# PrimeIntellect-ai/protocol

Measured on AMD Instinct MI355X. Metric: task x worker pair-evals/sec (full-swarm match), higher is better.
Workload: dtype u64

## Files before the change

protocol_amd/csrc/pm_device.h:

```cpp
#ifndef PM_DEVICE_H
#define PM_DEVICE_H

#include <hip/hip_runtime.h>
#include <stdint.h>

#include "pm_engine.h"

namespace pm {

static constexpr double PM_RAD = 3.14159265358979323846 / 180.0;
static constexpr uint64_t PM_KEY_NOLOC = 0x7FEFFFFFFFFFFFFFull;
static constexpr double PM_A_MAX_SAFE = 1.0 - 1.0 / 1048576.0;
static constexpr double PM_A_CHORD_MIN = 1.3e-6;
static constexpr uint32_t PM_CARVE_SLOTS = 8192;
static constexpr uint32_t PM_CARVE_PART = 64;
static constexpr uint32_t PM_CARVE_SEL_CAP = 256;
static constexpr uint32_t PM_CARVE_SLOT_BITS = 13;
static constexpr uint32_t PM_CARVE_BIG_SLOTS = 262144;
static constexpr uint32_t PM_CARVE_SLOT_BITS_BIG = 18;
static constexpr uint32_t PM_CARVE_SLOT_BITS_MEM = 21;
static constexpr double PM_TIE_BAND = 1.0 / 68719476736.0;
static constexpr double PM_TIE_BAND_BIG = 1.0 / 2147483648.0;
static constexpr double PM_TIE_BAND_MEM = 1.0 / 268435456.0;
static constexpr uint32_t PM_PROP_ROW = 96;
// ... 35 lines not shown
       SC_FINISH = 50,
       SC_FINISH_TICKET = 52,
       SC_TRACE = 51,
       SC_BATCHES = 54
};
static constexpr uint32_t PM_STREAM_TRACE_CAP = 1u << 17;
enum { SROW_NONE = 0, SROW_BITMAP = 1, SROW_WALK = 2, SROW_SWEEP = 3 };

struct CompatArgs {
  uint32_t W, n_cfgs, model_words;
  const uint32_t *flags, *gpu_count, *gpu_mem, *gpu_cls, *cpu_cores, *ram, *storage;
  const pm_config_row* cfgs;
  const pm_gpu_alt_row* alts;
  const uint32_t* model_bits;
  uint64_t* compat;
};

enum : uint32_t {
  REP_WHY = 0,
  REP_IDLE = PM_WHY_N,
  REP_GROUPS,
  REP_MEMBERS,
  REP_NO_TASK,
  REP_TASKS,
  REP_STRIDE = 16
};

struct ReportArgs {
  CompatArgs c;
  const int32_t* group_of;
// ... 196 lines not shown
  uint32_t stage_cap_g, stage_cap_m;
  uint32_t *stage_cfg, *stage_n, *stage_off, *stage_mem;
  unsigned long long* g_id_out;
  uint32_t* g_task_out;
  CarveStatus* h_status;
  unsigned long long* stream_trace;
  uint32_t n_avail, start_ci;
  uint32_t avail_cfg[PM_MAX_CONFIGS];
  uint32_t min_size[PM_MAX_CONFIGS];
  uint32_t max_size[PM_MAX_CONFIGS];
  uint32_t *g_cfg, *g_n, *g_off, *members;
  uint32_t cap_groups, cap_members;
  CarveStatus* status;
};

void launch_compat(const CompatArgs& a, hipStream_t s);
void launch_explain(const CompatArgs& p, const uint32_t* rows, uint32_t n, uint32_t stride, uint32_t* why_out, hipStream_t s);
void launch_config_report(const ReportArgs& a, uint32_t max_blocks, hipStream_t s);
void launch_task_report(const ReportArgs& a, uint32_t max_blocks, hipStream_t s);
void launch_group_spread(const SpreadArgs& a, hipStream_t s);
void launch_config_spread(const pm_group_spread_row* rows, const uint32_t* row_cfg, uint32_t n_rows, uint32_t n_cfgs,
                          SpreadCfgAcc* out, uint32_t max_blocks, hipStream_t s);
void launch_nearest(const NearArgs& a, hipStream_t s);
void launch_geo(const double* lat, const double* lon, double* coslat, double* ux, double* uy, double* uz, uint32_t W,
                hipStream_t s);
void launch_triad(const double* b, const double* c, double* a, size_t n, hipStream_t s);
#ifdef PM_ROW_BENCH
hipError_t launch_row_bench(const CarveArgs* d_args, uint32_t seed, uint32_t ci, uint32_t reps, uint32_t mode, unsigned long long* d_out, hipStream_t s);
#endif
void launch_row_network_test(const uint64_t* keys, const uint32_t* sites, uint32_t n_waves, uint32_t n_per_wave, uint32_t slot_bits,
                             uint64_t ulps, uint32_t upto, uint64_t* rows_out, uint32_t* mismatches, hipStream_t s);
// ... 1 lines not shown
void launch_distance_key_test(const double* in, const double* geo, uint32_t n, uint32_t mode, double* out, hipStream_t s);
void launch_update_rows(const RowUpdateArgs& a, hipStream_t s);
void launch_worker_selector(const int32_t* group_of, const uint32_t* g_cfg, uint32_t R, const uint32_t* rows,
                            uint64_t* sel, hipStream_t s);
void launch_eligible_selector(const uint32_t* wflags, const int32_t* group_of, const uint64_t* compat,
                              uint64_t enabled, uint32_t W, const uint8_t* shard, uint32_t my_rank, uint64_t* sel,
                              hipStream_t s);
void launch_chooser_rank(const int32_t* group_of, const uint64_t* g_id, const uint32_t* count, uint32_t R,
                         const uint32_t* rows, uint64_t seed, uint32_t* rank, hipStream_t s);
void launch_table_scatter(const pm_assignment* x, const uint32_t* xrow, uint32_t W, pm_assignment* table,
                          uint32_t* task_col, uint32_t* g_task_next, const uint64_t* t_live, const uint32_t* t_prefix,
                          hipStream_t s);
void launch_group_rank(const int32_t* group_of, const uint32_t* g_n, const uint32_t* g_off, const uint32_t* members,
                       const uint32_t* addr_rank, uint32_t W, uint32_t* rank_in_group, uint32_t* by_rank,
                       hipStream_t s);
void launch_claim_publish(const ClaimArgs& a, hipStream_t s);
void launch_match_prep(const MatchPrepArgs& a, hipStream_t s);
void launch_build_planes(const uint64_t* col_mask, uint32_t n_cols, uint32_t c_begin, uint32_t c_end, uint32_t stride,
                         uint32_t n_planes, uint64_t* planes, hipStream_t s);
void launch_pair_sweep(int variant, const uint64_t* row_sel, uint32_t R, const uint64_t* col_mask,
                       const uint64_t* planes, uint32_t c_begin, uint32_t c_end, uint32_t stride, uint32_t n_planes,
                       uint32_t* first, uint32_t* count, hipStream_t s, bool inited = false);
void launch_pair_select(int variant, const uint64_t* row_sel, uint32_t R, const uint64_t* col_mask,
                        const uint64_t* planes, uint32_t c_begin, uint32_t c_end, uint32_t stride, uint32_t n_planes,
                        const uint32_t* rank, uint32_t* out, hipStream_t s);
void launch_task_prefix(const uint64_t* live, uint32_t w_begin, uint32_t w_end, uint32_t* prefix, hipStream_t s);
void launch_task_delete(const uint32_t* slots, uint32_t n, uint64_t* tmask, uint64_t* live, uint64_t* planes,
                        uint32_t stride, uint32_t n_planes, hipStream_t s);
void launch_task_intern(const uint64_t* tmask, const uint64_t* live, uint32_t u_begin, uint32_t u_end, uint64_t valid,
                        uint64_t* keys, uint32_t n_slots, uint32_t* vals, uint32_t* counter_and_overflow, uint64_t* umask,
                        uint32_t cap_u, hipStream_t s);
// ... 3 lines not shown
                               uint32_t* count_out, hipStream_t s);
void launch_task_compact(const uint32_t* first_u, const uint32_t* count_u, uint32_t u_begin, uint32_t u_end,
                         const uint64_t* live, const uint32_t* prefix, uint32_t* first_out, uint32_t* count_out,
                         hipStream_t s);
void launch_newest(const int64_t* created_at, const uint64_t* live, uint32_t t_begin, uint32_t t_end,
                   uint32_t* idx_by_block, long long* val_by_block, uint32_t n_blocks, hipStream_t s);
void launch_group_ids(uint64_t* g_id, uint32_t* g_task, uint32_t n, uint64_t rng_state, hipStream_t s);
hipError_t carve_kernels_init();
hipError_t launch_carve(const CarveArgs* d_args, uint32_t flags, uint32_t start_ci, size_t lds_bytes, hipStream_t s);
uint32_t launch_carve_prep(const CarveArgs* d_args, uint32_t W, hipStream_t s);
hipError_t launch_carve_args_put(const CarveArgs& a, CarveArgs* d_args, hipStream_t s);
uint32_t launch_carve_elig(CarveArgs* d_args, const CarveArgs* put, uint32_t W, uint32_t n_bound, uint32_t index_min, uint32_t start_ci,
                           bool fresh, uint32_t n_groups0, uint32_t n_members0, hipStream_t s);
void launch_carve_apply(const CarveArgs* d_args, uint32_t W, hipStream_t s);
void launch_carve_propose(const CarveArgs* d_args, uint32_t W, hipStream_t s);
hipError_t launch_carve_stream(const CarveArgs* d_args, uint32_t start_ci, uint32_t n_prop_wgs, hipStream_t s);
void launch_scatter_const(uint32_t* dst, const uint32_t* idx, uint32_t n, uint32_t v, hipStream_t s);
void launch_scatter_pairs(uint32_t* dst, const uint32_t* pairs, uint32_t n, hipStream_t s);
void launch_merge_place(const CarveArgs* d_args, uint32_t n_order, uint32_t n_groups0, uint32_t n_members0, uint32_t steps0,
                        hipStream_t s);

}
#endif
```

protocol_amd/csrc/pm_engine_carve.inc:

```
static int32_t ensure_compat(pm_engine* e, hipEvent_t end_ev = nullptr) {
  if (!e->have_cfgs || !e->have_workers) return set_error(PM_ESTATE, "configs and workers must be uploaded first");
  {
    int32_t rcf = sync_flags(e);
    if (rcf) return rcf;
  }
  if (!e->compat_dirty) return PM_OK;
  for (const pm_gpu_alt_row& a : e->alts)
    if ((a.flags & PM_G_MODEL) && a.model_row >= e->model_rows)
      return set_error(PM_ESTATE, "a GPU alternative names a model row but pm_set_model_table was not called");
  if (e->model_rows && e->cls_check_dirty)
    for (uint32_t w = 0; w < e->W; ++w)
      if ((e->h_flags[w] & PM_W_GPU_MODEL) && e->h_gpu_cls[w] >= e->model_classes)
        return set_error(PM_ERANGE, "worker gpu_model_class outside the model table");
  e->cls_check_dirty = false;
  HIPCHK(e->d_compat.ensure(std::max<size_t>(e->W, 1)));
  CompatArgs a{};
  a.W = e->W;
  a.n_cfgs = uint32_t(e->cfgs.size());
  a.model_words = (e->model_classes + 31u) / 32u;
  a.flags = e->d_flags.p;
  a.gpu_count = e->d_gpu_count.p;
  a.gpu_mem = e->d_gpu_mem.p;
  a.gpu_cls = e->d_gpu_cls.p;
  a.cpu_cores = e->d_cpu_cores.p;
  a.ram = e->d_ram.p;
  a.storage = e->d_storage.p;
  a.cfgs = e->d_cfgs.p;
  a.alts = e->d_alts.p;
  a.model_bits = e->d_model_bits.p;
  a.compat = e->d_compat.p;
  HIPCHK(hipEventRecord(e->kev[0], e->stream));
  launch_compat(a, e->stream);
  HIPCHK(hipEventRecord(end_ev ? end_ev : e->kev[1], e->stream));
  HIPCHK(hipGetLastError());
  e->k_compat_recorded = true;
  e->k_compat_end = end_ev ? end_ev : e->kev[1];
  e->compat_dirty = false;
  e->h_compat_valid = false;
  return PM_OK;
}

static int32_t pull_compat(pm_engine* e) {
  if (e->h_compat_valid) return PM_OK;
  e->h_compat.resize(e->W);
  if (e->W) {
    HIPCHK(hipMemcpyAsync(e->h_compat.data(), e->d_compat.p, size_t(e->W) * 8, hipMemcpyDeviceToHost, e->stream));
    HIPCHK(hipStreamSynchronize(e->stream));
  }
  e->h_compat_valid = true;
  return PM_OK;
}
// ... 275 lines not shown
struct FormRun {
  CarveArgs a;
  CarveStatus st;
  std::vector<uint32_t> avail;
  uint32_t g0 = 0, m0 = 0, start_ci = 0;
  size_t lds = 0;
  bool use_props = false;
  bool nothing = false;
  uint32_t n_bound = 0;
  uint32_t n_elig_hint = 0;
  bool stream = false;
  uint32_t stream_wgs = 0;
  bool rearmed = false;
  uint32_t stage_cap = 0;
  bool args_pending = false;
};

static int32_t launch_propose_timed(pm_engine* e, const CarveArgs* d_args, uint32_t n_bound, hipStream_t s);

static int32_t form_setup_args(pm_engine* e, FormRun* r);

static int32_t form_queue_init(pm_engine* e, FormRun* r, bool fresh = false) {
  fresh = fresh && r->use_props;
  if (!fresh) HIPCHK(hipMemcpyAsync(e->d_status.p, &r->st, sizeof(r->st), hipMemcpyHostToDevice, e->stream));
  if (r->use_props) {
    if (!r->stream) HIPCHK(hipMemsetAsync(e->d_desc.p, 0, sizeof(BatchDesc), e->stream));
    const uint32_t index_min = !r->a.prune_mode ? 0u : r->a.prune_mode >= 2u ? 1u : PM_CELL_AUTO_N;
    if (r->stream) {
      if (e->stream_seq == 0 || e->stream_seq >= 127) {
        HIPCHK(hipMemsetAsync(e->d_stream_sq.p, 0, size_t(PM_STREAM_SQ) * 8, e->stream));
// ... 3 lines not shown
      }
      e->stream_seq += 1;
      const uint32_t tag0 = e->stream_seq << 25;
      if (r->a.stream_tag0 != tag0) {
        r->a.stream_tag0 = tag0;
        if (!r->args_pending)
          HIPCHK(hipMemcpyAsync(&e->d_carve_args.p->stream_tag0, &r->a.stream_tag0, sizeof(uint32_t), hipMemcpyHostToDevice, e->stream));
      }
    }
    e->tick_carve_launches += launch_carve_elig(e->d_carve_args.p, r->args_pending ? &r->a : nullptr, e->W, r->n_bound,
                                                r->n_elig_hint >= index_min ? index_min : 0u, r->start_ci, fresh, r->st.n_groups,
                                                r->st.n_members, e->stream);
    r->args_pending = false;
    host_mark("form: eligible list queued");
    if (r->stream) {
      HIPCHK(launch_carve_stream(e->d_carve_args.p, r->start_ci, r->stream_wgs, e->stream));
      e->tick_carve_launches += 2;
      return PM_OK;
    }
    e->tick_carve_launches += launch_carve_prep(e->d_carve_args.p, r->n_bound, e->stream);
    HIPCHK(hipGetLastError());
  } else
    HIPCHK(launch_carve(e->d_carve_args.p, CARVE_F_INIT | CARVE_F_RUN | CARVE_F_ALL, r->start_ci, r->lds, e->stream));
  e->tick_carve_launches++;
  return PM_OK;
}

static int32_t form_begin(pm_engine* e, FormRun* r, hipEvent_t begin_ev = nullptr) {
  int32_t rc = absorb_groups(e);
  if (rc) return rc;
  rc = ensure_compat(e);
// ... 292 lines not shown
```

protocol_amd/csrc/pm_engine_groups.inc:

```

template <typename T>
static int32_t upload(DevBuf<T>& d, const T* src, size_t n, hipStream_t s) {
  HIPCHK(d.ensure(n ? n : 1));
  if (n) HIPCHK(hipMemcpyAsync(d.p, src, n * sizeof(T), hipMemcpyHostToDevice, s));
  return PM_OK;
}

static void pub_clear(pm_engine* e) {
  const int cur = e->pub_cur.load(std::memory_order_relaxed);
  if (cur < 0) return;
  PubTable& t = e->pub[cur];
  const uint64_t s0 = t.seq.load(std::memory_order_relaxed);
  t.seq.store(s0 + 1, std::memory_order_relaxed);
  std::atomic_thread_fence(std::memory_order_release);
  t.cleared.store(1u, std::memory_order_relaxed);
  t.seq.store(s0 + 2, std::memory_order_release);
}

static void reset_groups_locked(pm_engine* e) {
  e->groups.clear();
  e->n_dead_groups = 0;
  e->absorb_pending = false;
  e->h_group_of.assign(e->W, -1);
  e->id_rng = e->cfg.group_id_seed;
// ... 40 lines not shown

static int32_t delta_stage(pm_engine* e, int which, size_t n) {
  HIPCHK(hipStreamSynchronize(e->stream));
  if (e->h_delta_cap[which] < n) {
    if (e->h_delta_pin[which]) (void)hipHostFree(e->h_delta_pin[which]);
    e->h_delta_pin[which] = nullptr;
    e->h_delta_cap[which] = 0;
    const size_t cap = n + n / 2 + 4096;
    HIPCHK(hipHostMalloc((void**)&e->h_delta_pin[which], cap * sizeof(uint32_t)));
    e->h_delta_cap[which] = cap;
  }
  HIPCHK(e->d_delta[which].ensure(n));
  return PM_OK;
}

static int32_t push_groups(pm_engine* e) {
  if (!e->groups_dirty) return PM_OK;
  const size_t room_g = std::min(e->d_g_cfg.cap, std::min(e->d_g_task.cap, std::min(e->d_g_task_next.cap, e->d_g_id.cap)));
  const size_t room_m = std::min(e->d_members.cap, std::min(e->d_by_rank.cap, e->d_rank_in_group.cap));
  if (e->groups_delta_ok && e->n_dead_groups * 4 <= e->groups.size() + 256 && size_t(e->d_n_groups) + e->W <= room_g &&
      size_t(e->d_n_members) + e->W <= room_m && e->d_n_groups == e->groups.size()) {
    HIPCHK(e->d_group_of.grow_keep(std::max<size_t>(e->W, 1), e->delta_tail_from == PM_NONE ? e->W : e->delta_tail_from, e->stream));
    if (e->delta_tail_from != PM_NONE && e->delta_tail_from < e->W)
      HIPCHK(hipMemsetAsync(e->d_group_of.p + e->delta_tail_from, 0xFF, size_t(e->W - e->delta_tail_from) * 4, e->stream));
    if (!e->delta_free.empty()) {
      const size_t n = e->delta_free.size();
      int32_t rc = delta_stage(e, 0, n);
      if (rc) return rc;
      std::memcpy(e->h_delta_pin[0], e->delta_free.data(), n * 4);
      HIPCHK(hipMemcpyAsync(e->d_delta[0].p, e->h_delta_pin[0], n * 4, hipMemcpyHostToDevice, e->stream));
      launch_scatter_const(reinterpret_cast<uint32_t*>(e->d_group_of.p), e->d_delta[0].p, uint32_t(n), 0xFFFFFFFFu, e->stream);
// ... 29 lines not shown
  HIPCHK(e->d_g_id.ensure(capG));
  HIPCHK(e->d_members.ensure(capM));
  HIPCHK(e->d_by_rank.ensure(capM));
  HIPCHK(e->d_rank_in_group.ensure(capM));
  HIPCHK(e->d_group_of.ensure(capM));
  if (G) {
    HIPCHK(hipMemcpyAsync(e->d_g_cfg.p, g_cfg.data(), G * 4, hipMemcpyHostToDevice, e->stream));
    HIPCHK(hipMemcpyAsync(e->d_g_n.p, g_n.data(), G * 4, hipMemcpyHostToDevice, e->stream));
    HIPCHK(hipMemcpyAsync(e->d_g_off.p, g_off.data(), G * 4, hipMemcpyHostToDevice, e->stream));
    HIPCHK(hipMemcpyAsync(e->d_g_task.p, g_task.data(), G * 4, hipMemcpyHostToDevice, e->stream));
    HIPCHK(hipMemcpyAsync(e->d_g_id.p, g_id.data(), G * 8, hipMemcpyHostToDevice, e->stream));
  }
  if (!members.empty())
    HIPCHK(hipMemcpyAsync(e->d_members.p, members.data(), members.size() * 4, hipMemcpyHostToDevice, e->stream));
  if (e->W) {
    if (G == 0)
      HIPCHK(hipMemsetAsync(e->d_group_of.p, 0xFF, size_t(e->W) * 4, e->stream));
    else
      HIPCHK(hipMemcpyAsync(e->d_group_of.p, e->h_group_of.data(), size_t(e->W) * 4, hipMemcpyHostToDevice, e->stream));
  }
  if (G) HIPCHK(hipStreamSynchronize(e->stream));
  e->d_n_groups = uint32_t(G);
  e->d_n_members = uint32_t(members.size());
  e->groups_dirty = false;
  e->groups_delta_ok = true;
  e->delta_free.clear();
  e->delta_tail_from = PM_NONE;
  return PM_OK;
}

static int32_t sync_flags(pm_engine* e) {
// ... 25 lines not shown
```

protocol_amd/csrc/pm_engine_match.inc:

```

static int32_t ensure_task_planes(pm_engine* e) {
  if (!e->have_tasks) return set_error(PM_ESTATE, "tasks must be uploaded first");
  const uint32_t n_planes = uint32_t(e->cfgs.size());
  const uint32_t stride = e->t_cap / 64u;
  if (e->tplanes_dirty) {
    HIPCHK(e->d_tplanes.ensure(std::max<size_t>(size_t(stride) * (n_planes + 1), 1)));
    launch_build_planes(e->d_tmask.p, e->t_cap, e->t_lo, e->t_cap, stride, n_planes, e->d_tplanes.p, e->stream);
    HIPCHK(hipGetLastError());
    e->tplanes_dirty = false;
  }
  if (e->tprefix_dirty) {
    launch_task_prefix(e->d_tlive.p, e->t_lo / 64u, stride, e->d_tprefix.p, e->stream);
    HIPCHK(hipGetLastError());
    e->tprefix_dirty = false;
  }
  return PM_OK;
}

static uint32_t task_position(pm_engine* e, uint32_t u) {
  if (u == PM_NONE || u < e->t_lo || u >= e->t_cap) return PM_NONE;
  if (!e->h_tprefix_valid) {
    const uint32_t stride = e->t_cap / 64u;
    e->h_tprefix.assign(stride, 0);
    uint32_t acc = 0;
// ... 34 lines not shown
  if (!n_app) return PM_OK;
  const uint64_t bit = 1ull << cfg;
  uint32_t r = 0;
  if (e->cfg.chooser == PM_CHOOSE_SEEDED) r = uint32_t(splitmix64_mix(e->cfg.chooser_seed ^ group_id) % n_app);
  for (uint32_t u = e->t_lo; u < e->t_cap; ++u)
    if (e->h_tmask[u] & bit) {
      if (r == 0) {
        *task_out = u;
        return PM_OK;
      }
      --r;
    }
  return PM_OK;
}

static int32_t run_match(pm_engine* e, bool want_count, std::vector<uint32_t>* count_out, bool dist = false, size_t G_ub = 0) {
  pm_assignment* const claim_h_table = dist ? nullptr : e->claim_h_table;
  uint32_t* const claim_h_gtask = dist ? nullptr : e->claim_h_gtask;
  e->claim_h_table = nullptr;
  e->claim_h_gtask = nullptr;
  if (!e->have_cfgs || !e->have_workers || !e->have_tasks)
    return set_error(PM_ESTATE, "configs, workers and tasks must be uploaded first");
  int32_t rc = push_groups(e);
  if (rc) return rc;
  const int variant = int(e->cfg.sweep_variant);
  host_mark("match: groups pushed");
  rc = ensure_task_planes(e);
  if (rc) return rc;
  host_mark("match: task planes");
  const uint32_t R = dist ? uint32_t(e->h_own_rows.size()) : e->W;
  const uint32_t* rows = dist ? e->d_own_rows.p : nullptr;
  rc = ensure_sweep_outputs(e, R);
  if (rc) return rc;
  HIPCHK(e->d_sel.ensure(std::max<uint32_t>(e->W, 1)));
  HIPCHK(e->d_table.ensure(std::max<uint32_t>(e->W, 1)));
  HIPCHK(e->d_task_col.ensure(std::max<uint32_t>(e->W, 1)));
  if (e->W == 0) return PM_OK;
  const uint32_t n_planes = uint32_t(e->cfgs.size());

  host_mark("match: selector launch");
  const size_t G = G_ub ? G_ub : e->d_n_groups;
  if (!dist) {
    MatchPrepArgs m{};
    m.W = e->W;
    m.G = uint32_t(G);
    m.group_of = e->d_group_of.p;
    m.g_cfg = e->d_g_cfg.p;
    m.g_n = e->d_g_n.p;
    m.g_off = e->d_g_off.p;
    m.members = e->d_members.p;
    m.addr_rank = e->d_addr_rank.p;
    m.g_task = e->d_g_task.p;
// ... 33 lines not shown
  c.group_of = e->d_group_of.p;
  c.g_n = e->d_g_n.p;
  c.g_off = e->d_g_off.p;
  c.g_task = e->d_g_task.p;
  c.g_id = e->d_g_id.p;
  c.g_task_next = e->d_g_task_next.p;
  c.chosen = chosen;
  c.rank_in_group = e->d_rank_in_group.p;
  c.by_rank = e->d_by_rank.p;
  c.t_live = e->d_tlive.p;
  c.t_prefix = e->d_tprefix.p;
  c.table = dist ? e->d_table_x.p + size_t(e->dist_rank) * e->dist_cap_t : e->d_table.p;
  c.task_col = e->d_task_col.p;
  c.h_table = claim_h_table;
  c.h_gtask = claim_h_gtask;
  launch_claim_publish(c, e->stream);
  HIPCHK(hipGetLastError());
  if (want_count && count_out) {
    count_out->resize(R);
    HIPCHK(hipMemcpyAsync(count_out->data(), e->d_count.p, size_t(R) * 4, hipMemcpyDeviceToHost, e->stream));
  }
  return PM_OK;
}

static int32_t pub_buffer(pm_engine* e, PubTable& t, uint32_t rows, uint64_t** out) {
  uint64_t* words = t.words.load(std::memory_order_relaxed);
  if (t.cap_rows < rows || !words) {
    const size_t cap = std::max<size_t>(size_t(rows) + rows / 8 + 64, 64);
    uint64_t* nw = nullptr;
    if (hipHostMalloc((void**)&nw, cap * 32) != hipSuccess || !nw)
      return set_error(PM_ENOMEM, "out of pinned host memory for the published table");
// ... 206 lines not shown
```

protocol_amd/csrc/pm_engine_state.inc:

```
struct pm_engine {
  pm_engine_config cfg{};
  hipStream_t stream = nullptr;
  hipStream_t stream_owned = nullptr;
  bool own_stream = true;
  hipEvent_t ev[6]{};
  hipEvent_t kev[6]{};
  hipEvent_t k_carve_begin = nullptr;
  hipEvent_t k_compat_end = nullptr;
  bool one_event_behind_carve = false;
  float k_ms_compat = 0, k_ms_carve = 0, k_ms_sweep = 0;
  bool k_sweep_recorded = false, k_compat_recorded = false;
  std::chrono::steady_clock::time_point tick_t0{};
  bool end_event_queued = false;
  uint64_t tick_cand_sum = 0;
  unsigned long long carve_prof[64]{};
  unsigned long long carve_why[25]{};
  uint32_t debug_mem_above = 0;
  uint32_t debug_abort_after = 0;
  uint32_t delta_pushes = 0;
  uint32_t merge_streamed = 0;
  uint32_t merge_stream_min = 512;
  uint32_t prune_mode = 1;
  uint32_t prune_factor = 512;
  uint32_t walk_cap_div = 0;
// ... 162 lines not shown
```

protocol_amd/csrc/pm_engine_tick.inc:

```
static void tick_reset(pm_engine* e) {
  e->tick_host_resolved = e->tick_carve_launches = e->tick_carve_steps = 0;
  e->tick_fast_steps = 0;
  e->tick_cand_sum = 0;
  e->tick_props = 0;
  e->tick_prop_keys = 0;
  e->tick_stream_timeouts = e->tick_stream_tickets = e->tick_stream_aborts = 0;
  e->k_ms_propose = 0;
  e->prop_ev_used = 0;
  e->k_ms_compat = e->k_ms_carve = e->k_ms_sweep = 0;
  e->k_sweep_recorded = e->k_compat_recorded = false;
  e->one_event_behind_carve = false;
  e->end_event_queued = false;
  e->tick_t0 = std::chrono::steady_clock::now();
}

static int32_t tick_stats(pm_engine* e, pm_stats* stats, uint32_t n_formed, uint32_t n_merged) {
  if (!e->end_event_queued) HIPCHK(hipEventRecord(e->ev[5], e->stream));
  HIPCHK(hipEventSynchronize(e->ev[5]));
  hipEvent_t const sweep_end = e->end_event_queued ? e->ev[5] : e->ev[4];
  pm_stats s{};
  HIPCHK(hipEventElapsedTime(&s.ms_compat, e->ev[0], e->ev[1]));
  HIPCHK(hipEventElapsedTime(&s.ms_carve, e->ev[1], e->ev[2]));
  if (e->one_event_behind_carve) {
    s.ms_merge = 0.0f;
    HIPCHK(hipEventElapsedTime(&s.ms_sweep, e->ev[2], sweep_end));
  } else {
    HIPCHK(hipEventElapsedTime(&s.ms_merge, e->ev[2], e->ev[3]));
    HIPCHK(hipEventElapsedTime(&s.ms_sweep, e->ev[3], sweep_end));
  }
  if (!e->end_event_queued) HIPCHK(hipEventElapsedTime(&s.ms_publish, e->ev[4], e->ev[5]));
  if (e->end_event_queued)
    s.ms_total = std::chrono::duration<float, std::milli>(std::chrono::steady_clock::now() - e->tick_t0).count();
  else
    HIPCHK(hipEventElapsedTime(&s.ms_total, e->ev[0], e->ev[5]));
  if (e->k_compat_recorded) HIPCHK(hipEventElapsedTime(&s.ms_compat_kernel, e->kev[0], e->k_compat_end ? e->k_compat_end : e->kev[1]));
  if (e->k_sweep_recorded) HIPCHK(hipEventElapsedTime(&s.ms_sweep_kernel, e->kev[4], e->kev[5]));
  s.ms_carve_kernel = e->k_ms_carve;
  s.carve_cand_sum = e->tick_cand_sum;
  s.ms_propose_kernel = e->k_ms_propose;
  s.proposals = e->tick_props;
  s.propose_keys = e->tick_prop_keys;
  s.n_groups = uint32_t(e->groups.size() - e->n_dead_groups);
  s.n_formed = n_formed;
  s.n_merged = n_merged;
  s.carve_steps = e->tick_carve_steps;
  s.carve_fast_steps = e->tick_fast_steps;
  s.host_resolved_steps = e->tick_host_resolved;
  s.carve_launches = e->tick_carve_launches;
  s.pair_evals = uint64_t(e->T) * uint64_t(e->W);
  e->last_stats = s;
// ... 1 lines not shown
  return PM_OK;
}

int32_t pm_tick(pm_engine* e, pm_stats* stats) {
  if (!e) return set_error(PM_EINVAL, "null argument");
  std::lock_guard<std::mutex> lk(e->mu);
  if (e->dist_phase != 0) return set_error(PM_ESTATE, "a stepwise tick is in progress");
  HIPCHK(hipSetDevice(e->cfg.device));
  if (!e->have_cfgs || !e->have_workers || !e->have_tasks)
    return set_error(PM_ESTATE, "configs, workers and tasks must be uploaded first");
  if (e->dist_world > 1) return set_error(PM_ESTATE, "multi-GPU engine: use the stepwise tick (pm_dist_tick_begin ...)");
  if (e->dist_phase != 0) return set_error(PM_ESTATE, "a stepwise tick is in progress");
  tick_reset(e);
  host_mark("tick: begin");
  uint32_t n_formed = 0, n_merged = 0;
  HIPCHK(hipEventRecord(e->ev[0], e->stream));
  e->compat_dirty = true;
  int32_t rc = absorb_groups(e);
  if (rc) return rc;
  rc = push_groups(e);
  if (rc) return rc;
  rc = ensure_task_planes(e);
  if (rc) return rc;
  rc = ensure_compat(e, e->ev[1]);
  if (rc) return rc;
  if (!e->k_compat_recorded) HIPCHK(hipEventRecord(e->ev[1], e->stream));
  host_mark("tick: compat queued");
  FormRun r;
  rc = form_begin(e, &r, e->ev[1]);
  if (rc) return rc;
  bool done = false;
  if (r.stream && !r.nothing && !e->tick_needs_merge) {
    PubRun pr;
    HIPCHK(hipEventRecord(e->ev[2], e->stream));
    const size_t G_ub = std::min<size_t>(size_t(r.g0) + r.stage_cap, std::min(e->d_g_task.cap, e->d_g_task_next.cap));
    host_mark("tick: carve queued");
    rc = publish_open(e, &pr, G_ub);
    if (rc) return rc;
    host_mark("tick: snapshot buffer open");
    rc = run_match(e, false, nullptr, false, G_ub);
    if (rc) {
      publish_abandon(e, pr);
      return rc;
    }
    HIPCHK(hipEventRecord(e->ev[5], e->stream));
    e->end_event_queued = true;
    host_mark("tick: everything queued");
    if (hipEventSynchronize(e->ev[2]) != hipSuccess) {
      publish_abandon(e, pr);
      return set_error(PM_ENODEV, "tick: the stream failed");
    }
    host_mark("tick: carve through");
    const CarveStatus& hs = *e->h_status;
    size_t solo = hs.n_solo;
    for (const Group& g : e->groups) solo += g.members.size() == 1 && !g.dead;
    const bool fits = hs.n_groups >= r.g0 && hs.n_groups - r.g0 <= r.stage_cap && hs.n_members >= r.m0 &&
                      hs.n_members - r.m0 <= r.stage_cap && hs.n_groups <= G_ub;
    if (hs.state == CARVE_STATE_DONE && fits && solo < 2) {
      r.st = hs;
      rc = form_finish(e, &r, &n_formed, false, true);
// ... 170 lines not shown
```

protocol_amd/csrc/pm_kernels.hip:

```cpp
#include <hip/hip_runtime.h>
#include <stdint.h>

#include "pm_device.h"

#if defined(__HIP_DEVICE_COMPILE__) && !defined(__gfx950__)
#error "pm_kernels.hip is written for gfx950 (MI355X): see the note on the placement kernels' fences above"
#endif

namespace pm {


template <int CTRL, int ROW_MASK>
__device__ __forceinline__ uint32_t dpp_add_step(uint32_t v) {
  return v + (uint32_t)__builtin_amdgcn_update_dpp(0, (int)v, CTRL, ROW_MASK, 0xF, false);
}
__device__ __forceinline__ uint32_t wave_incl_scan_u32(uint32_t v) {
  v = dpp_add_step<0x111, 0xF>(v);
  v = dpp_add_step<0x112, 0xF>(v);
  v = dpp_add_step<0x114, 0xF>(v);
  v = dpp_add_step<0x118, 0xF>(v);
  v = dpp_add_step<0x142, 0xA>(v);
  v = dpp_add_step<0x143, 0xC>(v);
  return v;
}
// ... 91 lines not shown
      }
      if ((cfg.flags & PM_R_RAM) && (!(wf & PM_W_RAM) || wram < cfg.ram_mb)) ok = false;
      if ((cfg.flags & PM_R_STORAGE) && (!(wf & PM_W_STORAGE) || wsto < cfg.storage_gb)) ok = false;
      if (cfg.alt_count) {
        bool any = false;
        if (wf & PM_W_HAS_GPU)
          for (uint32_t k = 0; k < cfg.alt_count; ++k)
            any |= gpu_alt_meets(wf, wcount, wmem, wcls, p.alts[cfg.alt_begin + k], p.model_bits, p.model_words);
        ok = ok && any;
      }
    }
    mask |= (uint64_t)ok << c;
  }
  if (!SLICED) {
    p.compat[w] = mask;
    return;
  }
  s_part[threadIdx.x] = mask;
  __syncthreads();
  if (slice == 0u && in) p.compat[w] = s_part[lane] | s_part[64u + lane] | s_part[128u + lane] | s_part[192u + lane];
}
__global__ __launch_bounds__(256) void compat_kernel(CompatArgs p) { compat_body<false>(p); }
__global__ __launch_bounds__(256) void compat_sliced_kernel(CompatArgs p) { compat_body<true>(p); }

__global__ __launch_bounds__(256) void triad_kernel(const double* __restrict__ b, const double* __restrict__ c,
                                                    double* __restrict__ a, size_t n) {
  for (size_t i = (size_t)blockIdx.x * 256u + threadIdx.x; i < n; i += (size_t)gridDim.x * 256u) a[i] = b[i] + 3.0 * c[i];
}

__device__ __forceinline__ void geo_of(double la, double lo, double* coslat, double* ux, double* uy, double* uz) {
  const double phi = la * PM_RAD, lam = lo * PM_RAD;
  const double c = cos(phi);
  *coslat = c;
  *ux = c * cos(lam);
  *uy = c * sin(lam);
// ... 530 lines not shown
```

protocol_amd/csrc/pm_launch.inc:

```

void launch_compat(const CompatArgs& a, hipStream_t s) {
  if (a.W == 0) return;
  if (a.W < 65536u)
    hipLaunchKernelGGL(compat_sliced_kernel, dim3((a.W + 63u) / 64u), dim3(256), 0, s, a);
  else
    hipLaunchKernelGGL(compat_kernel, dim3((a.W + 255u) / 256u), dim3(256), 0, s, a);
}
void launch_triad(const double* b, const double* c, double* a, size_t n, hipStream_t s) {
  hipLaunchKernelGGL(triad_kernel, dim3(256 * 32), dim3(256), 0, s, b, c, a, n);
}
void launch_row_network_test(const uint64_t* keys, const uint32_t* sites, uint32_t n_waves, uint32_t n_per_wave, uint32_t slot_bits,
                             uint64_t ulps, uint32_t upto, uint64_t* rows_out, uint32_t* mismatches, hipStream_t s) {
  hipLaunchKernelGGL(row_network_test_kernel, dim3(n_waves / 4u), dim3(256), 0, s, keys, sites, n_per_wave, slot_bits, ulps, upto, rows_out,
                     mismatches);
}
void launch_distance_key_test(const double* in, const double* geo, uint32_t n, uint32_t mode, double* out, hipStream_t s) {
  if (n == 0) return;
  hipLaunchKernelGGL(distance_key_test_kernel, dim3((n + 255u) / 256u), dim3(256), 0, s, in, geo, n, mode, out);
}
void launch_geo(const double* lat, const double* lon, double* coslat, double* ux, double* uy, double* uz, uint32_t W,
                hipStream_t s) {
  if (W == 0) return;
  hipLaunchKernelGGL(geo_kernel, dim3((W + 255u) / 256u), dim3(256), 0, s, lat, lon, coslat, ux, uy, uz, W);
}
// ... 26 lines not shown
  hipLaunchKernelGGL(table_scatter_kernel, dim3((W + 255u) / 256u), dim3(256), 0, s, x, xrow, W, table, task_col,
                     g_task_next, t_live, t_prefix);
}
void launch_group_rank(const int32_t* group_of, const uint32_t* g_n, const uint32_t* g_off, const uint32_t* members,
                       const uint32_t* addr_rank, uint32_t W, uint32_t* rank_in_group, uint32_t* by_rank,
                       hipStream_t s) {
  if (W == 0) return;
  hipLaunchKernelGGL(group_rank_kernel, dim3((W + 255u) / 256u), dim3(256), 0, s, group_of, g_n, g_off, members,
                     addr_rank, W, rank_in_group, by_rank);
}
void launch_match_prep(const MatchPrepArgs& a, hipStream_t s) {
  const uint32_t n = a.W > a.G ? a.W : a.G;
  if (n == 0) return;
  hipLaunchKernelGGL(match_prep_kernel, dim3((n + 255u) / 256u), dim3(256), 0, s, a);
}
void launch_claim_publish(const ClaimArgs& a, hipStream_t s) {
  if (a.R == 0) return;
  hipLaunchKernelGGL(claim_publish_kernel, dim3((a.R + 255u) / 256u), dim3(256), 0, s, a);
}

void launch_build_planes(const uint64_t* col_mask, uint32_t n_cols, uint32_t c_begin, uint32_t c_end, uint32_t stride,
                         uint32_t n_planes, uint64_t* planes, hipStream_t s) {
  const uint32_t w0 = c_begin / 64u, w1 = (c_end + 63u) / 64u;
  if (w1 <= w0) return;
  hipLaunchKernelGGL(build_planes_kernel, dim3(((w1 - w0) * 64u + 255u) / 256u), dim3(256), 0, s, col_mask, n_cols, w0,
                     w1, stride, n_planes, planes);
}

void launch_pair_sweep(int variant, const uint64_t* row_sel, uint32_t R, const uint64_t* col_mask,
                       const uint64_t* planes, uint32_t c_begin, uint32_t c_end, uint32_t stride, uint32_t n_planes,
                       uint32_t* first, uint32_t* count, hipStream_t s, bool inited) {
  if (R == 0) return;
  const uint32_t rb = (R + 255u) / 256u;
// ... 209 lines not shown
```

protocol_amd/csrc/pm_stream.inc:

```

enum { SLW_TREQ = PM_STREAM_TP,
       SLW_PAY,
       SLW_TISSUED,
       SLW_SCANW, SLW_SCANLO, SLW_SCANHI,
       SLW_TIMEOUTS,
       SLW_LA,
       SLW_TEND,
       SLW_ACKT, SLW_ACKP0, SLW_ACKP1, SLW_ACKP2, SLW_ACKP3, SLW_ACKP4,
       SLW_NCAND,
       SLW_P_CI, SLW_P_CI1, SLW_P_PAY, SLW_P_PAY1, SLW_P_MAX, SLW_P_MAX1, SLW_P_T0, SLW_P_T01, SLW_P_CNT, SLW_P_CNT1,
       SLW_P_SCANW, SLW_P_SCANW1, SLW_P_SCANLO, SLW_P_SCANLO1, SLW_P_SCANHI, SLW_P_SCANHI1,
       SLW_WORDS };
static_assert(SLW_TREQ == PM_STREAM_SLW_TREQ && SLW_PAY == PM_STREAM_SLW_PAY, "the words carve_fast_steps reads");
static_assert(SLW_WORDS <= PM_STREAM_TP + 32u, "ticket state fits its LDS region");
#ifndef STREAM_NPARK
#define STREAM_NPARK 5u
#endif
#ifndef STREAM_PARK_NB
#define STREAM_PARK_NB 16u
#endif
#ifndef STREAM_NAP_TICKETER
#define STREAM_NAP_TICKETER 4
#endif
#ifndef STREAM_NAP_PARK
// ... 2106 lines not shown
    st->fast_steps += c.fast_steps;
    st->slow_steps += c.steps - c.fast_steps;
    st->n_batches += 1u;
    if (n > 0u && n <= PM_CARVE_BIG_SLOTS) {
      st->stream_timeouts += sl_words[SLW_TIMEOUTS];
      st->stream_tickets += sl_words[SLW_TISSUED];
    }
  }
}

__global__ __launch_bounds__(256) void carve_finish_kernel(const CarveArgs* __restrict__ pa) {
  const CarveArgs& p = *pa;
  const auto st = G(p.status);
  const auto ctl = G(p.stream_ctl);
  __shared__ uint32_t s_last;
  if (ctl[SC_FINISH]) {
    const uint32_t g_lo = st->g_lo, g_hi = st->g_hi;
    const uint32_t total = gridDim.x * 256u;
    const uint32_t id_g0 = p.id_g0, m0 = p.stage_m0, cap_g = p.stage_cap_g, cap_m = p.stage_cap_m;
    const bool stage = p.stage_cfg != nullptr;
    uint32_t solo = 0;
    for (uint32_t g = g_lo + blockIdx.x * 256u + threadIdx.x; g < g_hi; g += total) {
      const uint32_t off = G(p.g_off)[g], gn = G(p.g_n)[g];
      const uint32_t k = g - id_g0;
      for (uint32_t j = 0; j < gn; ++j) {
        const uint32_t w = G(p.order)[G(p.members)[off + j]];
        G(p.members)[off + j] = w;
        if (p.mode == CARVE_MODE_FORM) G(p.group_of)[w] = (int32_t)g;
        if (stage && off + j - m0 < cap_m) p.stage_mem[off + j - m0] = w;
      }
      if (p.g_id_out) {
        unsigned long long z = p.id_state + (unsigned long long)(k + 1u) * 0x9E3779B97F4A7C15ull;
        z = (z ^ (z >> 30)) * 0xBF58476D1CE4E5B9ull;
        z = (z ^ (z >> 27)) * 0x94D049BB133111EBull;
        p.g_id_out[g] = z ^ (z >> 31);
        p.g_task_out[g] = PM_NONE;
      }
      if (stage && k < cap_g) {
        p.stage_cfg[k] = G(p.g_cfg)[g];
        p.stage_n[k] = gn;
        p.stage_off[k] = off;
      }
      solo += gn == 1u ? 1u : 0u;
    }
    solo = wave_sum(solo);
    if ((threadIdx.x & 63u) == 0u && solo) atomicAdd(&p.status->n_solo, solo);
  }
  if (!p.h_status) return;
  __syncthreads();
  if (threadIdx.x == 0) {
    __threadfence();
    s_last = atomicAdd(&p.stream_ctl[SC_FINISH_TICKET], 1u);
  }
  __syncthreads();
  if (s_last != gridDim.x - 1u) return;
  const auto src = G((const uint32_t*)p.status);
  uint32_t* dst = (uint32_t*)p.h_status;
  for (uint32_t k = threadIdx.x; k < (uint32_t)(sizeof(CarveStatus) / 4u); k += 256u) dst[k] = ld_ag32((const stream_gu32*)(src + k));
}

hipError_t launch_carve_stream(const CarveArgs* d_args, uint32_t start_ci, uint32_t n_prop_wgs, hipStream_t s) {
  hipLaunchKernelGGL(carve_stream_kernel, dim3(1u + n_prop_wgs), dim3(CARVE_THREADS), PM_STREAM_LDS_BYTES, s, d_args, start_ci);
  hipLaunchKernelGGL(carve_finish_kernel, dim3(128), dim3(256), 0, s, d_args);
  return hipGetLastError();
}

#ifdef PM_ROW_BENCH
__global__ __launch_bounds__(CARVE_THREADS) void carve_row_bench_kernel(const CarveArgs* __restrict__ pa, uint32_t s, uint32_t ci, uint32_t reps,
                                                                        unsigned long long* __restrict__ out) {
  const CarveArgs& p = *pa;
  extern __shared__ __attribute__((aligned(16))) unsigned char s_raw[];
  const uint32_t lane = threadIdx.x & 63u, wave = threadIdx.x >> 6;
  if (wave != 0u) return;
  const auto st = G((const CarveStatus*)p.status);
  const uint32_t n = st->n_eligible;
  if (n == 0u || n > PM_CARVE_BIG_SLOTS || s >= n) return;
  const uint32_t SB = n > PM_CARVE_SLOTS ? PM_CARVE_SLOT_BITS_BIG : PM_CARVE_SLOT_BITS;
  const double TIE_BAND = n > PM_CARVE_SLOTS ? PM_TIE_BAND_BIG : PM_TIE_BAND;
// ... 42 lines not shown
```

Measured before the change: 1130 billion.

## Fold group_of reset into compat kernel, attach events to launches, parallelize member finish

The separate memset that resets group_of to -1 is folded into the compat kernel, and standalone hipEventRecord calls are replaced by events attached to hipExtLaunchKernelGGL launches, cutting commands on the stream per tick. The carve finish kernel also moves member remapping from a per-group serial loop to a per-member loop, where each block locates its group by cooperative binary search over g_off. This balances work when group sizes vary, at the cost of extra searches and block barriers. The ev[0] record now moves to the compat launch, so the total-time window measured from ev[0] shrinks.

```diff
diff --git a/protocol_amd/csrc/pm_device.h b/protocol_amd/csrc/pm_device.h
--- a/protocol_amd/csrc/pm_device.h
+++ b/protocol_amd/csrc/pm_device.h
@@ -73,6 +73,7 @@
   const pm_gpu_alt_row* alts;
   const uint32_t* model_bits;
   uint64_t* compat;
+  int32_t* group_of_fill;
 };
 
 enum : uint32_t {
@@ -299,7 +300,7 @@
   CarveStatus* status;
 };
 
-void launch_compat(const CompatArgs& a, hipStream_t s);
+bool launch_compat(const CompatArgs& a, hipStream_t s, hipEvent_t start_ev = nullptr, hipEvent_t stop_ev = nullptr);
 void launch_explain(const CompatArgs& p, const uint32_t* rows, uint32_t n, uint32_t stride, uint32_t* why_out, hipStream_t s);
 void launch_config_report(const ReportArgs& a, uint32_t max_blocks, hipStream_t s);
 void launch_task_report(const ReportArgs& a, uint32_t max_blocks, hipStream_t s);
@@ -331,7 +332,7 @@
 void launch_group_rank(const int32_t* group_of, const uint32_t* g_n, const uint32_t* g_off, const uint32_t* members,
                        const uint32_t* addr_rank, uint32_t W, uint32_t* rank_in_group, uint32_t* by_rank,
                        hipStream_t s);
-void launch_claim_publish(const ClaimArgs& a, hipStream_t s);
+bool launch_claim_publish(const ClaimArgs& a, hipStream_t s, hipEvent_t stop_ev = nullptr);
 void launch_match_prep(const MatchPrepArgs& a, hipStream_t s);
 void launch_build_planes(const uint64_t* col_mask, uint32_t n_cols, uint32_t c_begin, uint32_t c_end, uint32_t stride,
                          uint32_t n_planes, uint64_t* planes, hipStream_t s);
@@ -365,7 +366,7 @@
                            bool fresh, uint32_t n_groups0, uint32_t n_members0, hipStream_t s);
 void launch_carve_apply(const CarveArgs* d_args, uint32_t W, hipStream_t s);
 void launch_carve_propose(const CarveArgs* d_args, uint32_t W, hipStream_t s);
-hipError_t launch_carve_stream(const CarveArgs* d_args, uint32_t start_ci, uint32_t n_prop_wgs, hipStream_t s);
+hipError_t launch_carve_stream(const CarveArgs* d_args, uint32_t start_ci, uint32_t n_prop_wgs, hipStream_t s, hipEvent_t finish_ev = nullptr);
 void launch_scatter_const(uint32_t* dst, const uint32_t* idx, uint32_t n, uint32_t v, hipStream_t s);
 void launch_scatter_pairs(uint32_t* dst, const uint32_t* pairs, uint32_t n, hipStream_t s);
 void launch_merge_place(const CarveArgs* d_args, uint32_t n_order, uint32_t n_groups0, uint32_t n_members0, uint32_t steps0,
diff --git a/protocol_amd/csrc/pm_engine_carve.inc b/protocol_amd/csrc/pm_engine_carve.inc
--- a/protocol_amd/csrc/pm_engine_carve.inc
+++ b/protocol_amd/csrc/pm_engine_carve.inc
@@ -1,4 +1,4 @@
-static int32_t ensure_compat(pm_engine* e, hipEvent_t end_ev = nullptr) {
+static int32_t ensure_compat(pm_engine* e, hipEvent_t begin_ev = nullptr, hipEvent_t end_ev = nullptr) {
   if (!e->have_cfgs || !e->have_workers) return set_error(PM_ESTATE, "configs and workers must be uploaded first");
   {
     int32_t rcf = sync_flags(e);
@@ -29,12 +29,25 @@
   a.alts = e->d_alts.p;
   a.model_bits = e->d_model_bits.p;
   a.compat = e->d_compat.p;
-  HIPCHK(hipEventRecord(e->kev[0], e->stream));
-  launch_compat(a, e->stream);
-  HIPCHK(hipEventRecord(end_ev ? end_ev : e->kev[1], e->stream));
+  if (begin_ev && end_ev) {
+    if (e->group_of_fill_pending) a.group_of_fill = e->d_group_of.p;
+    if (launch_compat(a, e->stream, begin_ev, end_ev)) {
+      e->group_of_fill_pending = false;
+    } else {
+      HIPCHK(hipEventRecord(begin_ev, e->stream));
+      HIPCHK(hipEventRecord(end_ev, e->stream));
+    }
+    e->k_compat_begin = begin_ev;
+    e->k_compat_end = end_ev;
+  } else {
+    HIPCHK(hipEventRecord(e->kev[0], e->stream));
+    launch_compat(a, e->stream);
+    HIPCHK(hipEventRecord(e->kev[1], e->stream));
+    e->k_compat_begin = e->kev[0];
+    e->k_compat_end = e->kev[1];
+  }
   HIPCHK(hipGetLastError());
   e->k_compat_recorded = true;
-  e->k_compat_end = end_ev ? end_ev : e->kev[1];
   e->compat_dirty = false;
   e->h_compat_valid = false;
   return PM_OK;
@@ -340,6 +353,7 @@
   bool rearmed = false;
   uint32_t stage_cap = 0;
   bool args_pending = false;
+  hipEvent_t finish_ev = nullptr;
 };
 
 static int32_t launch_propose_timed(pm_engine* e, const CarveArgs* d_args, uint32_t n_bound, hipStream_t s);
@@ -373,7 +387,7 @@
     r->args_pending = false;
     host_mark("form: eligible list queued");
     if (r->stream) {
-      HIPCHK(launch_carve_stream(e->d_carve_args.p, r->start_ci, r->stream_wgs, e->stream));
+      HIPCHK(launch_carve_stream(e->d_carve_args.p, r->start_ci, r->stream_wgs, e->stream, r->finish_ev));
       e->tick_carve_launches += 2;
       return PM_OK;
     }
diff --git a/protocol_amd/csrc/pm_engine_groups.inc b/protocol_amd/csrc/pm_engine_groups.inc
--- a/protocol_amd/csrc/pm_engine_groups.inc
+++ b/protocol_amd/csrc/pm_engine_groups.inc
@@ -78,7 +78,7 @@
   return PM_OK;
 }
 
-static int32_t push_groups(pm_engine* e) {
+static int32_t push_groups(pm_engine* e, bool fill_by_compat = false) {
   if (!e->groups_dirty) return PM_OK;
   const size_t room_g = std::min(e->d_g_cfg.cap, std::min(e->d_g_task.cap, std::min(e->d_g_task_next.cap, e->d_g_id.cap)));
   const size_t room_m = std::min(e->d_members.cap, std::min(e->d_by_rank.cap, e->d_rank_in_group.cap));
@@ -138,7 +138,9 @@
   if (!members.empty())
     HIPCHK(hipMemcpyAsync(e->d_members.p, members.data(), members.size() * 4, hipMemcpyHostToDevice, e->stream));
   if (e->W) {
-    if (G == 0)
+    if (G == 0 && fill_by_compat)
+      e->group_of_fill_pending = true;
+    else if (G == 0)
       HIPCHK(hipMemsetAsync(e->d_group_of.p, 0xFF, size_t(e->W) * 4, e->stream));
     else
       HIPCHK(hipMemcpyAsync(e->d_group_of.p, e->h_group_of.data(), size_t(e->W) * 4, hipMemcpyHostToDevice, e->stream));
diff --git a/protocol_amd/csrc/pm_engine_match.inc b/protocol_amd/csrc/pm_engine_match.inc
--- a/protocol_amd/csrc/pm_engine_match.inc
+++ b/protocol_amd/csrc/pm_engine_match.inc
@@ -72,7 +72,8 @@
   return PM_OK;
 }
 
-static int32_t run_match(pm_engine* e, bool want_count, std::vector<uint32_t>* count_out, bool dist = false, size_t G_ub = 0) {
+static int32_t run_match(pm_engine* e, bool want_count, std::vector<uint32_t>* count_out, bool dist = false, size_t G_ub = 0,
+                         hipEvent_t end_ev = nullptr) {
   pm_assignment* const claim_h_table = dist ? nullptr : e->claim_h_table;
   uint32_t* const claim_h_gtask = dist ? nullptr : e->claim_h_gtask;
   e->claim_h_table = nullptr;
@@ -93,7 +94,10 @@
   HIPCHK(e->d_sel.ensure(std::max<uint32_t>(e->W, 1)));
   HIPCHK(e->d_table.ensure(std::max<uint32_t>(e->W, 1)));
   HIPCHK(e->d_task_col.ensure(std::max<uint32_t>(e->W, 1)));
-  if (e->W == 0) return PM_OK;
+  if (e->W == 0) {
+    if (end_ev) HIPCHK(hipEventRecord(end_ev, e->stream));
+    return PM_OK;
+  }
   const uint32_t n_planes = uint32_t(e->cfgs.size());
 
   host_mark("match: selector launch");
@@ -157,7 +161,7 @@
   c.task_col = e->d_task_col.p;
   c.h_table = claim_h_table;
   c.h_gtask = claim_h_gtask;
-  launch_claim_publish(c, e->stream);
+  if (!launch_claim_publish(c, e->stream, end_ev) && end_ev) HIPCHK(hipEventRecord(end_ev, e->stream));
   HIPCHK(hipGetLastError());
   if (want_count && count_out) {
     count_out->resize(R);
diff --git a/protocol_amd/csrc/pm_engine_state.inc b/protocol_amd/csrc/pm_engine_state.inc
--- a/protocol_amd/csrc/pm_engine_state.inc
+++ b/protocol_amd/csrc/pm_engine_state.inc
@@ -7,6 +7,8 @@
   hipEvent_t kev[6]{};
   hipEvent_t k_carve_begin = nullptr;
   hipEvent_t k_compat_end = nullptr;
+  hipEvent_t k_compat_begin = nullptr;
+  bool group_of_fill_pending = false;
   bool one_event_behind_carve = false;
   float k_ms_compat = 0, k_ms_carve = 0, k_ms_sweep = 0;
   bool k_sweep_recorded = false, k_compat_recorded = false;
diff --git a/protocol_amd/csrc/pm_engine_tick.inc b/protocol_amd/csrc/pm_engine_tick.inc
--- a/protocol_amd/csrc/pm_engine_tick.inc
+++ b/protocol_amd/csrc/pm_engine_tick.inc
@@ -33,7 +33,7 @@
     s.ms_total = std::chrono::duration<float, std::milli>(std::chrono::steady_clock::now() - e->tick_t0).count();
   else
     HIPCHK(hipEventElapsedTime(&s.ms_total, e->ev[0], e->ev[5]));
-  if (e->k_compat_recorded) HIPCHK(hipEventElapsedTime(&s.ms_compat_kernel, e->kev[0], e->k_compat_end ? e->k_compat_end : e->kev[1]));
+  if (e->k_compat_recorded) HIPCHK(hipEventElapsedTime(&s.ms_compat_kernel, e->k_compat_begin ? e->k_compat_begin : e->kev[0], e->k_compat_end ? e->k_compat_end : e->kev[1]));
   if (e->k_sweep_recorded) HIPCHK(hipEventElapsedTime(&s.ms_sweep_kernel, e->kev[4], e->kev[5]));
   s.ms_carve_kernel = e->k_ms_carve;
   s.carve_cand_sum = e->tick_cand_sum;
@@ -65,36 +65,38 @@
   tick_reset(e);
   host_mark("tick: begin");
   uint32_t n_formed = 0, n_merged = 0;
-  HIPCHK(hipEventRecord(e->ev[0], e->stream));
   e->compat_dirty = true;
   int32_t rc = absorb_groups(e);
   if (rc) return rc;
-  rc = push_groups(e);
+  rc = push_groups(e, true);
   if (rc) return rc;
   rc = ensure_task_planes(e);
   if (rc) return rc;
-  rc = ensure_compat(e, e->ev[1]);
-  if (rc) return rc;
-  if (!e->k_compat_recorded) HIPCHK(hipEventRecord(e->ev[1], e->stream));
+  rc = ensure_compat(e, e->ev[0], e->ev[1]);
+  if (e->group_of_fill_pending) {
+    e->group_of_fill_pending = false;
+    if (e->W && hipMemsetAsync(e->d_group_of.p, 0xFF, size_t(e->W) * 4, e->stream) != hipSuccess && !rc)
+      rc = set_error(PM_ENODEV, "tick: the stream failed");
+  }
+  if (rc) return rc;
   host_mark("tick: compat queued");
   FormRun r;
+  r.finish_ev = e->ev[2];
   rc = form_begin(e, &r, e->ev[1]);
   if (rc) return rc;
   bool done = false;
   if (r.stream && !r.nothing && !e->tick_needs_merge) {
     PubRun pr;
-    HIPCHK(hipEventRecord(e->ev[2], e->stream));
     const size_t G_ub = std::min<size_t>(size_t(r.g0) + r.stage_cap, std::min(e->d_g_task.cap, e->d_g_task_next.cap));
     host_mark("tick: carve queued");
     rc = publish_open(e, &pr, G_ub);
     if (rc) return rc;
     host_mark("tick: snapshot buffer open");
-    rc = run_match(e, false, nullptr, false, G_ub);
+    rc = run_match(e, false, nullptr, false, G_ub, e->ev[5]);
     if (rc) {
       publish_abandon(e, pr);
       return rc;
     }
-    HIPCHK(hipEventRecord(e->ev[5], e->stream));
     e->end_event_queued = true;
     host_mark("tick: everything queued");
     if (hipEventSynchronize(e->ev[2]) != hipSuccess) {
diff --git a/protocol_amd/csrc/pm_kernels.hip b/protocol_amd/csrc/pm_kernels.hip
--- a/protocol_amd/csrc/pm_kernels.hip
+++ b/protocol_amd/csrc/pm_kernels.hip
@@ -1,4 +1,5 @@
 #include <hip/hip_runtime.h>
+#include <hip/hip_ext.h>
 #include <stdint.h>
 
 #include "pm_device.h"
@@ -129,11 +130,13 @@
   }
   if (!SLICED) {
     p.compat[w] = mask;
+    if (p.group_of_fill) p.group_of_fill[w] = -1;
     return;
   }
   s_part[threadIdx.x] = mask;
   __syncthreads();
   if (slice == 0u && in) p.compat[w] = s_part[lane] | s_part[64u + lane] | s_part[128u + lane] | s_part[192u + lane];
+  if (slice == 1u && in && p.group_of_fill) p.group_of_fill[w] = -1;
 }
 __global__ __launch_bounds__(256) void compat_kernel(CompatArgs p) { compat_body<false>(p); }
 __global__ __launch_bounds__(256) void compat_sliced_kernel(CompatArgs p) { compat_body<true>(p); }
diff --git a/protocol_amd/csrc/pm_launch.inc b/protocol_amd/csrc/pm_launch.inc
--- a/protocol_amd/csrc/pm_launch.inc
+++ b/protocol_amd/csrc/pm_launch.inc
@@ -1,10 +1,11 @@
 
-void launch_compat(const CompatArgs& a, hipStream_t s) {
-  if (a.W == 0) return;
+bool launch_compat(const CompatArgs& a, hipStream_t s, hipEvent_t start_ev, hipEvent_t stop_ev) {
+  if (a.W == 0) return false;
   if (a.W < 65536u)
-    hipLaunchKernelGGL(compat_sliced_kernel, dim3((a.W + 63u) / 64u), dim3(256), 0, s, a);
+    hipExtLaunchKernelGGL(compat_sliced_kernel, dim3((a.W + 63u) / 64u), dim3(256), 0, s, start_ev, stop_ev, 0, a);
   else
-    hipLaunchKernelGGL(compat_kernel, dim3((a.W + 255u) / 256u), dim3(256), 0, s, a);
+    hipExtLaunchKernelGGL(compat_kernel, dim3((a.W + 255u) / 256u), dim3(256), 0, s, start_ev, stop_ev, 0, a);
+  return true;
 }
 void launch_triad(const double* b, const double* c, double* a, size_t n, hipStream_t s) {
   hipLaunchKernelGGL(triad_kernel, dim3(256 * 32), dim3(256), 0, s, b, c, a, n);
@@ -64,9 +65,10 @@
   if (n == 0) return;
   hipLaunchKernelGGL(match_prep_kernel, dim3((n + 255u) / 256u), dim3(256), 0, s, a);
 }
-void launch_claim_publish(const ClaimArgs& a, hipStream_t s) {
-  if (a.R == 0) return;
-  hipLaunchKernelGGL(claim_publish_kernel, dim3((a.R + 255u) / 256u), dim3(256), 0, s, a);
+bool launch_claim_publish(const ClaimArgs& a, hipStream_t s, hipEvent_t stop_ev) {
+  if (a.R == 0) return false;
+  hipExtLaunchKernelGGL(claim_publish_kernel, dim3((a.R + 255u) / 256u), dim3(256), 0, s, nullptr, stop_ev, 0, a);
+  return true;
 }
 
 void launch_build_planes(const uint64_t* col_mask, uint32_t n_cols, uint32_t c_begin, uint32_t c_end, uint32_t stride,
diff --git a/protocol_amd/csrc/pm_stream.inc b/protocol_amd/csrc/pm_stream.inc
--- a/protocol_amd/csrc/pm_stream.inc
+++ b/protocol_amd/csrc/pm_stream.inc
@@ -2144,21 +2144,18 @@
   const auto st = G(p.status);
   const auto ctl = G(p.stream_ctl);
   __shared__ uint32_t s_last;
+  __shared__ uint32_t s_cnt[4];
+  __shared__ uint32_t s_goff[256], s_gn[256];
+  const uint32_t tid = threadIdx.x, lane = tid & 63u, wave = tid >> 6;
   if (ctl[SC_FINISH]) {
     const uint32_t g_lo = st->g_lo, g_hi = st->g_hi;
     const uint32_t total = gridDim.x * 256u;
     const uint32_t id_g0 = p.id_g0, m0 = p.stage_m0, cap_g = p.stage_cap_g, cap_m = p.stage_cap_m;
     const bool stage = p.stage_cfg != nullptr;
     uint32_t solo = 0;
-    for (uint32_t g = g_lo + blockIdx.x * 256u + threadIdx.x; g < g_hi; g += total) {
-      const uint32_t off = G(p.g_off)[g], gn = G(p.g_n)[g];
+    for (uint32_t g = g_lo + blockIdx.x * 256u + tid; g < g_hi; g += total) {
+      const uint32_t gn = G(p.g_n)[g];
       const uint32_t k = g - id_g0;
-      for (uint32_t j = 0; j < gn; ++j) {
-        const uint32_t w = G(p.order)[G(p.members)[off + j]];
-        G(p.members)[off + j] = w;
-        if (p.mode == CARVE_MODE_FORM) G(p.group_of)[w] = (int32_t)g;
-        if (stage && off + j - m0 < cap_m) p.stage_mem[off + j - m0] = w;
-      }
       if (p.g_id_out) {
         unsigned long long z = p.id_state + (unsigned long long)(k + 1u) * 0x9E3779B97F4A7C15ull;
         z = (z ^ (z >> 30)) * 0xBF58476D1CE4E5B9ull;
@@ -2169,16 +2166,52 @@
       if (stage && k < cap_g) {
         p.stage_cfg[k] = G(p.g_cfg)[g];
         p.stage_n[k] = gn;
-        p.stage_off[k] = off;
+        p.stage_off[k] = G(p.g_off)[g];
       }
       solo += gn == 1u ? 1u : 0u;
     }
     solo = wave_sum(solo);
-    if ((threadIdx.x & 63u) == 0u && solo) atomicAdd(&p.status->n_solo, solo);
+    if (lane == 0u && solo) atomicAdd(&p.status->n_solo, solo);
+    if (g_hi > g_lo) {
+      const uint32_t m_lo = G(p.g_off)[g_lo], m_hi = G(p.g_off)[g_hi - 1u] + G(p.g_n)[g_hi - 1u];
+      for (uint32_t mb = m_lo + blockIdx.x * 256u; mb < m_hi; mb += total) {
+        uint32_t lo = g_lo, hi = g_hi;
+        while (hi - lo > 1u) {
+          const uint32_t step = (hi - lo + 255u) / 256u;
+          const uint32_t g = lo + tid * step;
+          const bool ok = g < hi && G(p.g_off)[g] <= mb;
+          const uint32_t c = (uint32_t)__popcll(__ballot(ok));
+          __syncthreads();
+          if (lane == 0u) s_cnt[wave] = c;
+          __syncthreads();
+          const uint32_t n_ok = s_cnt[0] + s_cnt[1] + s_cnt[2] + s_cnt[3];
+          lo += (n_ok - 1u) * step;
+          hi = min(hi, lo + step);
+        }
+        __syncthreads();
+        s_goff[tid] = lo + tid < g_hi ? G(p.g_off)[lo + tid] : 0xFFFFFFFFu;
+        s_gn[tid] = lo + tid < g_hi ? G(p.g_n)[lo + tid] : 0u;
+        __syncthreads();
+        const uint32_t m = mb + tid;
+        if (m < m_hi) {
+          uint32_t a = 0u, b = 256u;
+          while (b - a > 1u) {
+            const uint32_t mid = (a + b) >> 1;
+            if (s_goff[mid] <= m) a = mid; else b = mid;
+          }
+          if (m - s_goff[a] < s_gn[a]) {
+            const uint32_t w = G(p.order)[G(p.members)[m]];
+            G(p.members)[m] = w;
+            if (p.mode == CARVE_MODE_FORM) G(p.group_of)[w] = (int32_t)(lo + a);
+            if (stage && m - m0 < cap_m) p.stage_mem[m - m0] = w;
+          }
+        }
+      }
+    }
   }
   if (!p.h_status) return;
   __syncthreads();
-  if (threadIdx.x == 0) {
+  if (tid == 0) {
     __threadfence();
     s_last = atomicAdd(&p.stream_ctl[SC_FINISH_TICKET], 1u);
   }
@@ -2186,12 +2219,15 @@
   if (s_last != gridDim.x - 1u) return;
   const auto src = G((const uint32_t*)p.status);
   uint32_t* dst = (uint32_t*)p.h_status;
-  for (uint32_t k = threadIdx.x; k < (uint32_t)(sizeof(CarveStatus) / 4u); k += 256u) dst[k] = ld_ag32((const stream_gu32*)(src + k));
+  for (uint32_t k = tid; k < (uint32_t)(sizeof(CarveStatus) / 4u); k += 256u) dst[k] = ld_ag32((const stream_gu32*)(src + k));
 }
 
-hipError_t launch_carve_stream(const CarveArgs* d_args, uint32_t start_ci, uint32_t n_prop_wgs, hipStream_t s) {
+hipError_t launch_carve_stream(const CarveArgs* d_args, uint32_t start_ci, uint32_t n_prop_wgs, hipStream_t s, hipEvent_t finish_ev) {
   hipLaunchKernelGGL(carve_stream_kernel, dim3(1u + n_prop_wgs), dim3(CARVE_THREADS), PM_STREAM_LDS_BYTES, s, d_args, start_ci);
-  hipLaunchKernelGGL(carve_finish_kernel, dim3(128), dim3(256), 0, s, d_args);
+  if (finish_ev)
+    hipExtLaunchKernelGGL(carve_finish_kernel, dim3(128), dim3(256), 0, s, nullptr, finish_ev, 0, d_args);
+  else
+    hipLaunchKernelGGL(carve_finish_kernel, dim3(128), dim3(256), 0, s, d_args);
   return hipGetLastError();
 }
 
```

After: 1143 billion, median of 6. About the same (+1.2%).
